# cwi-dis/cwipc_util

Hardware: NVIDIA B200
Metric: Mpoints/s for downsample+remove_outliers at 1/2/4/8 B200; % of HBM GB/s peak (higher is better)
Workload: dtype f32 keys/distances, int64 fixed-point sums, f64 statistics

## Files before the change

### cwipc_util_b200/csrc/outliers.cu

```cuda
#include <algorithm>
#include <cmath>
#include <cstdlib>
#include <cstring>
#include <mutex>

#include "device_utils.cuh"
#include "kernels.hpp"
#include "radix_sort.hpp"

namespace cwcu {

namespace {

constexpr int KG_MAX_LEVELS = 14;

struct GridParams {
    float gmin[3];
    float inv_h;
    float h;
    float rc;
    float rc_far;
    int second_min;
    int second_max;
    int gdim[3];
    int idxbits;
    int top_level;
    int bands;
    int band_bits;
    int xdim;
    uint32_t table_off[KG_MAX_LEVELS];
};
struct BandLut {
    uint8_t rank[256];
};

__host__ __device__ __forceinline__ int level_dim(int gdim, int level) { return ((gdim - 1) >> level) + 1; }

__device__ __forceinline__ uint32_t table_index(const GridParams &gp, int level, uint32_t x, uint32_t y, uint32_t z) {
    const uint32_t dx = (uint32_t)level_dim(gp.gdim[0], level), dy = (uint32_t)level_dim(gp.gdim[1], level);
    return gp.table_off[level] + (z * dy + y) * dx + x;
}

__device__ __forceinline__ uint64_t spread3(uint32_t v) {
    uint64_t x = v & 0x1fffffu;
    x = (x | x << 32) & 0x1f00000000ffffull;
    x = (x | x << 16) & 0x1f0000ff0000ffull;
    x = (x | x << 8) & 0x100f00f00f00f00full;
    x = (x | x << 4) & 0x10c30c30c30c30c3ull;
    x = (x | x << 2) & 0x1249249249249249ull;
    return x;
}
__device__ __forceinline__ uint32_t compact3(uint64_t x) {
    x &= 0x1249249249249249ull;
    x = (x | x >> 2) & 0x10c30c30c30c30c3ull;
    x = (x | x >> 4) & 0x100f00f00f00f00full;
    x = (x | x >> 8) & 0x1f0000ff0000ffull;
    x = (x | x >> 16) & 0x1f00000000ffffull;
    x = (x | x >> 32) & 0x1fffffull;
    return (uint32_t)x;
}
__device__ __forceinline__ uint64_t morton3(uint32_t x, uint32_t y, uint32_t z) { return (spread3(x) << 2) | (spread3(y) << 1) | spread3(z); }

__device__ __forceinline__ float cell_u(float x, float gmin, float inv_h) { return __fmul_rn(__fsub_rn(x, gmin), inv_h); }
__device__ __forceinline__ int cell_of(float u, int gdim) { return min(max((int)floorf(u), 0), gdim - 1); }

__device__ __forceinline__ float dist2(const Point16 &a, const Point16 &b) {
    const float dx = __fsub_rn(a.x, b.x), dy = __fsub_rn(a.y, b.y), dz = __fsub_rn(a.z, b.z);
    return __fadd_rn(__fadd_rn(__fmul_rn(dx, dx), __fmul_rn(dy, dy)), __fmul_rn(dz, dz));
}

__global__ void __launch_bounds__(256) knn_keygen_kernel(const cwipc_point *__restrict__ pts, uint32_t n, const __grid_constant__ GridParams gp, const __grid_constant__ BandLut lut,
                                                          uint64_t *__restrict__ keys, uint2 *__restrict__ table, uint32_t table_words2) {
    for (uint32_t i = blockIdx.x * blockDim.x + threadIdx.x; i < table_words2; i += gridDim.x * blockDim.x) table[i] = make_uint2(0u, 0u);
    for (uint32_t i = blockIdx.x * blockDim.x + threadIdx.x; i < n; i += gridDim.x * blockDim.x) {
        const Point16 p = ld_point_stream(pts, i);
        uint32_t cx = cell_of(cell_u(p.x, gp.gmin[0], gp.inv_h), gp.xdim);
        const uint32_t cy = cell_of(cell_u(p.y, gp.gmin[1], gp.inv_h), gp.gdim[1]);
        const uint32_t cz = cell_of(cell_u(p.z, gp.gmin[2], gp.inv_h), gp.gdim[2]);
        if (gp.bands > 1) cx += (uint32_t)lut.rank[pt_tile(p)] << gp.band_bits;
        keys[i] = (morton3(cx, cy, cz) << gp.idxbits) | i;
    }
}

__global__ void __launch_bounds__(256) knn_layout_kernel(const uint64_t *__restrict__ sorted, uint32_t n, GridParams gp, const cwipc_point *__restrict__ pts,
                                                          cwipc_point *__restrict__ spts, uint2 *__restrict__ table) {
    const uint64_t idxmask = (1ull << gp.idxbits) - 1ull;
    for (uint32_t i = blockIdx.x * blockDim.x + threadIdx.x; i < n; i += gridDim.x * blockDim.x) {
        const uint64_t word = sorted[i];
        st_point(spts, i, ld_point(pts, (size_t)(word & idxmask)));
        const uint64_t code = word >> gp.idxbits;
        int top;
        uint64_t prev = 0;
        if (i == 0) {
            top = gp.top_level;
        } else {
            prev = sorted[i - 1] >> gp.idxbits;
            const uint64_t diff = code ^ prev;
            top = diff ? min((63 - __clzll((long long)diff)) / 3, gp.top_level) : -1;
        }
        if (top >= 0) {
            const uint32_t cx = compact3(code >> 2), cy = compact3(code >> 1), cz = compact3(code);
            const uint32_t px = compact3(prev >> 2), py = compact3(prev >> 1), pz = compact3(prev);
            for (int l = 0; l <= top; l++) {
                table[table_index(gp, l, cx >> l, cy >> l, cz >> l)].x = i;
                if (i > 0) table[table_index(gp, l, px >> l, py >> l, pz >> l)].y = i;
            }
// ... 24 lines not shown
        if (!done) {
            if (t0 == 0) t0 = clock64();
            else if (clock64() - t0 > 4000000000ll) __trap();
        }
    } while (!done);
}
__device__ __forceinline__ void bulk_g2s(void *dst, const void *src, uint32_t bytes, uint64_t *bar) {
    asm volatile("cp.async.bulk.shared::cluster.global.mbarrier::complete_tx::bytes [%0], [%1], %2, [%3];" ::"r"(smem_u32(dst)), "l"(src), "r"(bytes),
                 "r"(smem_u32(bar))
                 : "memory");
}

template <int N>
__device__ __forceinline__ void bitonic_sort_asc(float (&a)[N]) {
#pragma unroll
    for (int k = 2; k <= N; k <<= 1) {
#pragma unroll
        for (int j = k >> 1; j > 0; j >>= 1) {
#pragma unroll
            for (int i = 0; i < N; i++) {
                const int l = i ^ j;
                if (l > i) {
                    const float lo = fminf(a[i], a[l]), hi = fmaxf(a[i], a[l]);
                    const bool up = (i & k) == 0;
                    a[i] = up ? lo : hi;
                    a[l] = up ? hi : lo;
                }
            }
        }
    }
}
template <int N>
__device__ __forceinline__ void bitonic_merge_asc(float (&a)[N]) {
#pragma unroll
    for (int j = N >> 1; j > 0; j >>= 1) {
#pragma unroll
        for (int i = 0; i < N; i++) {
            const int l = i ^ j;
            if (l > i) {
                const float lo = fminf(a[i], a[l]), hi = fmaxf(a[i], a[l]);
                a[i] = lo;
                a[l] = hi;
            }
        }
    }
}

struct FarEntry {
    uint32_t q;
    float bound;
};

constexpr int KT_WARPS = 2;
constexpr int KT_THREADS = KT_WARPS * 32;
constexpr int KT_CH = 128;
constexpr int KT_STAGES = 2;
constexpr int KT_GROUP_LEVEL = 2;
constexpr int KT_GROUP_SPAN = 1 << KT_GROUP_LEVEL;
constexpr int KT_MAXR = (KT_GROUP_SPAN + 2) * (KT_GROUP_SPAN + 2) * (KT_GROUP_SPAN + 2);
constexpr int KT_BUF = 16;
constexpr int KT_BLOCKS_PER_SM = 12;

struct __align__(128) KnnWarpSmem {
    Point16 cand[KT_STAGES][KT_CH];
    float buf[KT_BUF][32];
    uint2 ranges[KT_MAXR];
    uint64_t mbar[KT_STAGES];
    float pbox[7];
    uint32_t xoff;
    uint32_t cursor;
};

__device__ __forceinline__ float warp_min(float v) {
#pragma unroll
    for (int o = 16; o > 0; o >>= 1) v = fminf(v, __shfl_xor_sync(FULL_MASK, v, o));
    return v;
}
__device__ __forceinline__ float warp_max(float v) {
#pragma unroll
    for (int o = 16; o > 0; o >>= 1) v = fmaxf(v, __shfl_xor_sync(FULL_MASK, v, o));
    return v;
}

template <int KCAP>
__global__ void __launch_bounds__(KT_THREADS, KT_BLOCKS_PER_SM) knn_tile_kernel(const cwipc_point *__restrict__ spts, const uint64_t *__restrict__ sorted, uint32_t n, GridParams gp, int kk, int k,
                                                               const uint2 *__restrict__ table, float *__restrict__ dist_out, float *__restrict__ kth_out, uint32_t nquery,
                                                               FarEntry *__restrict__ far_list, uint32_t *__restrict__ far_count) {
    extern __shared__ __align__(128) unsigned char knn_smem_raw[];
    constexpr int B = KCAP < KT_BUF ? KCAP : KT_BUF;
    const unsigned lane = lane_id(), warp = threadIdx.x >> 5;
    KnnWarpSmem &ws = reinterpret_cast<KnnWarpSmem *>(knn_smem_raw)[warp];
    const unsigned lt = lanemask_lt();
    if (lane == 0) {
#pragma unroll
        for (int st = 0; st < KT_STAGES; st++) mbar_init(&ws.mbar[st], 1);
        mbar_fence_init();
    }
    __syncwarp();
    uint32_t phase_bits = 0;

    const uint32_t warps_total = (gridDim.x * blockDim.x) >> 5;
    const uint64_t idxmask = (1ull << gp.idxbits) - 1ull;
    const int extra = KCAP - kk;
    const uint32_t nitems = (n + 31u) >> 5;
    const Point16 *spts16 = reinterpret_cast<const Point16 *>(spts);
    const float rc = gp.rc;
    const float reach = (rc - 0.01f) * gp.h;
    const float reach2 = reach * reach * 0.999999f;

    for (uint32_t item = (blockIdx.x * blockDim.x + threadIdx.x) >> 5; item < nitems; item += warps_total) {
        const uint32_t qi = item * 32u + lane;
        const uint32_t qs = qi < n ? qi : n - 1u;
        const uint64_t word = sorted[qs];
        const bool active = qi < n && (uint32_t)(word & idxmask) < nquery;
        const uint64_t code = word >> gp.idxbits;
        const Point16 q = spts16[qs];
        const float ux = cell_u(q.x, gp.gmin[0], gp.inv_h), uy = cell_u(q.y, gp.gmin[1], gp.inv_h), uz = cell_u(q.z, gp.gmin[2], gp.inv_h);
        const uint32_t band = gp.bands > 1 ? (compact3(code >> 2) >> gp.band_bits) : 0u;

        const uint64_t node2 = code >> (3 * KT_GROUP_LEVEL);
        const uint64_t prev_node2 = __shfl_up_sync(FULL_MASK, node2, 1);
        const unsigned heads = __ballot_sync(FULL_MASK, (lane == 0) || (node2 != prev_node2));
        const int m = __popc(heads);
        const int ord = __popc(heads & (lt | (1u << lane))) - 1;

        for (int g = 0; g < m; g++) {
            const bool live = active && ord == g;

            const float lox = warp_min(live ? ux : INFINITY), loy = warp_min(live ? uy : INFINITY), loz = warp_min(live ? uz : INFINITY);
            const float hix = warp_max(live ? ux : -INFINITY), hiy = warp_max(live ? uy : -INFINITY), hiz = warp_max(live ? uz : -INFINITY);
            uint32_t nr = 0, total = 0;
            const uint32_t xoff = gp.bands > 1 ? (__reduce_max_sync(FULL_MASK, live ? band : 0u) << gp.band_bits) : 0u;
            if (lox <= hix) {
                const int cx0 = max((int)floorf(lox - rc), 0), cx1 = min((int)floorf(hix + rc), gp.xdim - 1);
                const int cy0 = max((int)floorf(loy - rc), 0), cy1 = min((int)floorf(hiy + rc), gp.gdim[1] - 1);
                const int cz0 = max((int)floorf(loz - rc), 0), cz1 = min((int)floorf(hiz + rc), gp.gdim[2] - 1);
                const int nbx = cx1 - cx0 + 1, nby = cy1 - cy0 + 1, nbz = cz1 - cz0 + 1;
                const int nb = nbx * nby * nbz;
                const float rc2 = rc * rc;
                for (int shell = 0; shell < 2; shell++) {
                    for (int t0 = 0; t0 < nb; t0 += 32) {
                        const int t = t0 + (int)lane;
                        uint2 r = make_uint2(0u, 0u);
                        if (t < nb) {
                            const int ix = cx0 + t % nbx, iy = cy0 + (t / nbx) % nby, iz = cz0 + t / (nbx * nby);
                            const float dx = fmaxf(fmaxf((float)ix - hix, lox - (float)(ix + 1)), 0.f);
                            const float dy = fmaxf(fmaxf((float)iy - hiy, loy - (float)(iy + 1)), 0.f);
                            const float dz = fmaxf(fmaxf((float)iz - hiz, loz - (float)(iz + 1)), 0.f);
                            const float dd = dx * dx + dy * dy + dz * dz;
                            if (shell == 0 ? dd == 0.f : (dd > 0.f && dd <= rc2)) r = table[table_index(gp, 0, (uint32_t)ix + xoff, (uint32_t)iy, (uint32_t)iz)];
                        }
                        const unsigned has = __ballot_sync(FULL_MASK, r.y > r.x);
                        if (r.y > r.x) ws.ranges[nr + __popc(has & lt)] = r;
                        nr += __popc(has);
                        total += warp_sum(r.y - r.x);
                    }
                }
            }
            __syncwarp();

            float best[KCAP];
#pragma unroll
            for (int j = 0; j < KCAP; j++) best[j] = (j < extra) ? -INFINITY : INFINITY;
            float tau = live ? INFINITY : -INFINITY;
            uint32_t bcnt = 0;

            const uint32_t nchunks = (total + KT_CH - 1) / KT_CH;
            uint32_t ri = 0, roff = 0;
            auto fill = [&](int st, uint32_t chunk) {
                const uint32_t cnt = min((uint32_t)KT_CH, total - chunk * KT_CH);
                mbar_arrive_expect_tx(&ws.mbar[st], cnt * 16u);
                uint32_t filled = 0;
                while (filled < cnt) {
                    const uint2 r = ws.ranges[ri];
                    const uint32_t len = r.y - r.x;
                    const uint32_t take = min(len - roff, cnt - filled);
                    bulk_g2s(&ws.cand[st][filled], spts16 + r.x + roff, take * 16u, &ws.mbar[st]);
                    filled += take;
                    roff += take;
                    if (roff == len) {
                        ri++;
                        roff = 0;
                    }
                }
            };
            if (lane == 0 && nchunks > 0) {
                fill(0, 0);
                if (nchunks > 1) fill(1, 1);
            }
            for (uint32_t chunk = 0; chunk < nchunks; chunk++) {
                const int st = (int)(chunk & 1u);
                mbar_wait(&ws.mbar[st], (phase_bits >> st) & 1u);
                phase_bits ^= 1u << st;
                const uint32_t cnt = min((uint32_t)KT_CH, total - chunk * KT_CH);
                const bool last_chunk = chunk + 1 == nchunks;
                for (uint32_t c = 0; c < cnt; c += 4) {
                    if (c + 4 <= cnt) {
#pragma unroll
                        for (int u = 0; u < 4; u++) {
                            const Point16 cand = ws.cand[st][c + u];
                            const float d2 = dist2(q, cand);
                            if (d2 < tau) {
                                ws.buf[bcnt][lane] = d2;
                                bcnt++;
                            }
                        }
                    } else {
                        for (uint32_t u = c; u < cnt; u++) {
                            const float d2 = dist2(q, ws.cand[st][u]);
                            if (d2 < tau) {
                                ws.buf[bcnt][lane] = d2;
                                bcnt++;
                            }
                        }
                    }
                    const bool finish = last_chunk && c + 4 >= cnt;
                    if (finish || __any_sync(FULL_MASK, bcnt > (uint32_t)(B - 4))) {
                        float s[B];
#pragma unroll
                        for (int j = 0; j < B; j++) s[j] = ((uint32_t)j < bcnt) ? ws.buf[j][lane] : INFINITY;
                        bitonic_sort_asc<B>(s);
#pragma unroll
                        for (int j = 0; j < B; j++) best[KCAP - 1 - j] = fminf(best[KCAP - 1 - j], s[j]);
                        bitonic_merge_asc<KCAP>(best);
                        bcnt = 0;
                        if (live) tau = best[KCAP - 1];
                    }
                }
                __syncwarp();
                if (lane == 0 && chunk + 2 < nchunks) fill(st, chunk + 2);
            }

            const float worst = best[KCAP - 1];
            const bool done = live && (gp.top_level == 0 || worst <= reach2);
            const unsigned fm = __ballot_sync(FULL_MASK, live && !done);
            if (fm) {
                uint32_t slot = 0;
                if (lane == (unsigned)(__ffs(fm) - 1)) slot = atomicAdd(far_count, (uint32_t)__popc(fm));
                slot = __shfl_sync(FULL_MASK, slot, __ffs(fm) - 1);
                if (live && !done) {
                    FarEntry e;
                    e.q = qi;
                    e.bound = worst;
                    far_list[slot + __popc(fm & lt)] = e;
                }
            }
            if (!done) continue;
            double sum = 0.0;
#pragma unroll
            for (int j = 0; j < KCAP; j++)
                if (j > extra) sum += sqrt((double)best[j]);
            dist_out[(size_t)(word & idxmask)] = (float)(sum / (double)k);
            if (kth_out) kth_out[(size_t)(word & idxmask)] = worst;
        }
        __syncwarp();
    }
}


template <int KCAP>
__global__ void __launch_bounds__(KT_THREADS, KT_BLOCKS_PER_SM) knn_second_kernel(const cwipc_point *__restrict__ spts, const uint64_t *__restrict__ sorted, GridParams gp, int kk, int k,
                                                                 const uint2 *__restrict__ table, float *__restrict__ dist_out, float *__restrict__ kth_out,
                                                                 const FarEntry *__restrict__ far_list, const uint32_t *__restrict__ far_count, uint32_t second_from,
                                                                 FarEntry *__restrict__ far_list2, uint32_t *__restrict__ far_count2) {
    extern __shared__ __align__(128) unsigned char knn_smem_raw[];
    constexpr int B = KCAP < KT_BUF ? KCAP : KT_BUF;
    const unsigned lane = lane_id(), warp = threadIdx.x >> 5;
    KnnWarpSmem &ws = reinterpret_cast<KnnWarpSmem *>(knn_smem_raw)[warp];
    const unsigned lt = lanemask_lt();
    if (lane == 0) {
#pragma unroll
        for (int st = 0; st < KT_STAGES; st++) mbar_init(&ws.mbar[st], 1);
        mbar_fence_init();
    }
    __syncwarp();
    uint32_t phase_bits = 0;

    const uint32_t warps_total = (gridDim.x * blockDim.x) >> 5;
    const uint64_t idxmask = (1ull << gp.idxbits) - 1ull;
    const int extra = KCAP - kk;
    const uint32_t nent = *far_count;
    if (nent < second_from) return;
    const uint32_t nitems = (nent + 31u) >> 5;
    const Point16 *spts16 = reinterpret_cast<const Point16 *>(spts);

    for (uint32_t item = (blockIdx.x * blockDim.x + threadIdx.x) >> 5; item < nitems; item += warps_total) {
        const uint32_t ei = item * 32u + lane;
        const bool valid = ei < nent;
        const FarEntry ent = far_list[valid ? ei : nent - 1u];
        const uint64_t word = sorted[ent.q];
        const uint64_t code = word >> gp.idxbits;
        const Point16 q = spts16[ent.q];
        const float need = sqrtf(ent.bound) * gp.inv_h * 1.000001f + 0.02f;
        const uint64_t node2 = code >> (3 * KT_GROUP_LEVEL);
        bool active = valid && need <= gp.rc_far;
        {
            const unsigned peers = __match_any_sync(FULL_MASK, node2) & __ballot_sync(FULL_MASK, active);
            active = active && __popc(peers) >= gp.second_min;
        }
        {
            const unsigned fm = __ballot_sync(FULL_MASK, valid && !active);
            if (fm) {
                uint32_t slot = 0;
                if (lane == (unsigned)(__ffs(fm) - 1)) slot = atomicAdd(far_count2, (uint32_t)__popc(fm));
                slot = __shfl_sync(FULL_MASK, slot, __ffs(fm) - 1);
                if (valid && !active) far_list2[slot + __popc(fm & lt)] = ent;
            }
        }
        if (!__any_sync(FULL_MASK, active)) continue;

        const uint64_t prev_node2 = __shfl_up_sync(FULL_MASK, node2, 1);
        const unsigned heads = __ballot_sync(FULL_MASK, (lane == 0) || (node2 != prev_node2));
        const int m = __popc(heads);
        const int ord = __popc(heads & (lt | (1u << lane))) - 1;

        for (int g = 0; g < m; g++) {
            const bool live = active && ord == g;
            if (!__any_sync(FULL_MASK, live)) continue;
            {
                const float ux = cell_u(q.x, gp.gmin[0], gp.inv_h), uy = cell_u(q.y, gp.gmin[1], gp.inv_h), uz = cell_u(q.z, gp.gmin[2], gp.inv_h);
                const float lx = warp_min(live ? ux : INFINITY), ly = warp_min(live ? uy : INFINITY), lz = warp_min(live ? uz : INFINITY);
                const float hx = warp_max(live ? ux : -INFINITY), hy = warp_max(live ? uy : -INFINITY), hz = warp_max(live ? uz : -INFINITY);
                const float pr = warp_max(live ? need : 0.f);
                const uint32_t band = gp.bands > 1 ? __reduce_max_sync(FULL_MASK, live ? (compact3(code >> 2) >> gp.band_bits) : 0u) : 0u;
                if (lane == 0) {
                    ws.pbox[0] = lx; ws.pbox[1] = ly; ws.pbox[2] = lz;
                    ws.pbox[3] = hx; ws.pbox[4] = hy; ws.pbox[5] = hz;
                    ws.pbox[6] = pr;
                    ws.xoff = band << gp.band_bits;
                    ws.cursor = 0u;
                }
            }
            __syncwarp();

            float best[KCAP];
#pragma unroll
            for (int j = 0; j < KCAP; j++) best[j] = (j < extra) ? -INFINITY : INFINITY;
            float tau = live ? __uint_as_float(__float_as_uint(ent.bound) + 1u) : -INFINITY;
// ... 347 lines not shown
        const int cl = node_level - 1;
        const uint32_t chx = 2u * node_x + ((lane >> 2) & 1u), chy = 2u * node_y + ((lane >> 1) & 1u), chz = 2u * node_z + (lane & 1u);
        push_nodes(expand, cl, chx, chy, chz, thr);
        __syncwarp();
    }
}

__global__ void __launch_bounds__(256) knn_queue_all_kernel(const uint64_t *__restrict__ sorted, uint32_t n, int idxbits, uint32_t nquery, FarEntry *__restrict__ far_list,
                                                             uint32_t *__restrict__ far_count) {
    const uint64_t idxmask = (1ull << idxbits) - 1ull;
    const unsigned lane = lane_id();
    const uint32_t rounds = (n + blockDim.x * gridDim.x - 1) / (blockDim.x * gridDim.x);
    for (uint32_t r = 0; r < rounds; r++) {
        const uint32_t i = (r * gridDim.x + blockIdx.x) * blockDim.x + threadIdx.x;
        const bool query = i < n && (uint32_t)(sorted[i] & idxmask) < nquery;
        const unsigned m = __ballot_sync(FULL_MASK, query);
        if (m == 0u) continue;
        uint32_t first = 0;
        if (lane == (unsigned)(__ffs(m) - 1)) first = atomicAdd(far_count, (uint32_t)__popc(m));
        first = __shfl_sync(FULL_MASK, first, __ffs(m) - 1);
        if (query) {
            FarEntry e;
            e.q = i;
            e.bound = INFINITY;
            far_list[first + __popc(m & lanemask_lt())] = e;
        }
    }
}

__device__ __forceinline__ FarStart far_start(const Point16 q, uint64_t code, const GridParams &gp, int kk, const uint2 *__restrict__ table, uint32_t band, float &limit) {
    const unsigned lane = lane_id();
    const uint32_t cx = compact3(code >> 2), cy = compact3(code >> 1), cz = compact3(code);
    const int root_level = gp.bands > 1 ? gp.band_bits : gp.top_level;
    const float slack = 0.01f * gp.h;
    const float qq[3] = {q.x, q.y, q.z};
    bool enough = false;
    float far2 = INFINITY;
    if ((int)lane <= root_level) {
        const int l = (int)lane;
        const uint32_t ax = cx >> l, ay = cy >> l, az = cz >> l;
        const uint2 r = table[table_index(gp, l, ax, ay, az)];
        if (r.y - r.x >= (uint32_t)kk) {
            enough = true;
            const float pitch = ldexpf(gp.h, l);
            const uint32_t lx = ax - (band << (gp.band_bits - l));
            const float lo[3] = {gp.gmin[0] + (float)lx * pitch, gp.gmin[1] + (float)ay * pitch, gp.gmin[2] + (float)az * pitch};
            far2 = 0.f;
#pragma unroll
            for (int a = 0; a < 3; a++) {
                const float d = fmaxf(qq[a] - lo[a], (lo[a] + pitch) - qq[a]) + slack;
                far2 += d * d;
            }
        }
    }
    FarStart st;
    st.level = -1;
    st.x = st.y = st.z = 0u;
    const unsigned m = __ballot_sync(FULL_MASK, enough);
    if (m != 0u) limit = fminf(limit, __shfl_sync(FULL_MASK, far2, __ffs(m) - 1) * 1.0001f);
    if (!(limit < INFINITY)) return st;
    const float rcells = sqrtf(limit) * gp.inv_h * 1.000001f + 0.02f;
    const float u[3] = {cell_u(q.x, gp.gmin[0], gp.inv_h), cell_u(q.y, gp.gmin[1], gp.inv_h), cell_u(q.z, gp.gmin[2], gp.inv_h)};
    const int dim[3] = {gp.xdim, gp.gdim[1], gp.gdim[2]};
    uint32_t lo[3], hi[3];
#pragma unroll
    for (int a = 0; a < 3; a++) {
        lo[a] = (uint32_t)min(max((int)floorf(u[a] - rcells), 0), dim[a] - 1);
        hi[a] = (uint32_t)min(max((int)floorf(u[a] + rcells), 0), dim[a] - 1);
    }
    lo[0] += band << gp.band_bits;
    hi[0] += band << gp.band_bits;
    for (int l = 0; l < root_level; l++) {
        if ((hi[0] >> l) - (lo[0] >> l) <= 1u && (hi[1] >> l) - (lo[1] >> l) <= 1u && (hi[2] >> l) - (lo[2] >> l) <= 1u) {
            st.level = l;
            st.x = lo[0] >> l;
            st.y = lo[1] >> l;
            st.z = lo[2] >> l;
            break;
        }
    }
    return st;
}

template <int KPL>
__global__ void __launch_bounds__(KF_THREADS) knn_far_kernel(const cwipc_point *__restrict__ spts, const uint64_t *__restrict__ sorted, uint32_t n, const __grid_constant__ GridParams gp, int kk, int k,
                                                              const uint2 *__restrict__ table, float *__restrict__ dist_out, float *__restrict__ kth_out,
                                                              const FarEntry *__restrict__ far_list, const uint32_t *__restrict__ far_count, uint32_t second_from,
                                                              uint32_t leaf_points, bool far_start_enabled) {
    __shared__ __align__(16) FarNode s_stack[KF_WARPS][KF_STACK];
    const unsigned lane = lane_id(), warp = threadIdx.x >> 5;
    if (far_count[0] >= second_from) {
        far_list += (size_t)n + 64;
        far_count += 1;
    }
    const uint32_t nentries = *far_count;
    const uint32_t warps_total = (gridDim.x * blockDim.x) >> 5;
    const uint64_t idxmask = (1ull << gp.idxbits) - 1ull;
    const Point16 *spts16 = reinterpret_cast<const Point16 *>(spts);
    for (uint32_t ei = (blockIdx.x * blockDim.x + threadIdx.x) >> 5; ei < nentries; ei += warps_total) {
        const FarEntry ent = far_list[ei];
        float v[KPL];
        const uint64_t code = sorted[ent.q] >> gp.idxbits;
        const uint32_t band = gp.bands > 1 ? (compact3(code >> 2) >> gp.band_bits) : 0u;
        const Point16 q = spts16[ent.q];
        float limit = ent.bound;
        FarStart start;
        start.level = -1;
        start.x = start.y = start.z = 0u;
        if (far_start_enabled) start = far_start(q, code, gp, kk, table, band, limit);
        dfs_knn<KPL>(q, limit, spts16, n, gp, kk, table, leaf_points, s_stack[warp], v, band, start);
        double sq[KPL];
#pragma unroll
        for (int j = 0; j < KPL; j++) sq[j] = sqrt((double)v[j]);
        double *s_sq = reinterpret_cast<double *>(s_stack[warp]);
        __syncwarp();
#pragma unroll
        for (int j = 0; j < KPL; j++) s_sq[j * 32 + (int)lane] = sq[j];
        __syncwarp();
        double sum = 0.0;
        for (int e = 1; e <= k; e++) sum += s_sq[e];
        const float kth = list_element<KPL>(v, kk - 1);
        __syncwarp();
        if (lane == 0) {
            const size_t orig = (size_t)(sorted[ent.q] & idxmask);
            dist_out[orig] = (float)(sum / (double)k);
            if (kth_out) kth_out[orig] = kth;
        }
    }
}

template <int KPL>
__global__ void __launch_bounds__(KF_THREADS) knn_list_kernel(const cwipc_point *__restrict__ spts, uint32_t n, GridParams gp, int kk, const uint2 *__restrict__ table,
                                                               const cwipc_point *__restrict__ queries, const float *__restrict__ limits, uint32_t nq, float *__restrict__ lists,
                                                               uint32_t leaf_points) {
    __shared__ __align__(16) FarNode s_stack[KF_WARPS][KF_STACK];
    const unsigned lane = lane_id(), warp = threadIdx.x >> 5;
    const uint32_t warps_total = (gridDim.x * blockDim.x) >> 5;
    const Point16 *spts16 = reinterpret_cast<const Point16 *>(spts);
    for (uint32_t qi = (blockIdx.x * blockDim.x + threadIdx.x) >> 5; qi < nq; qi += warps_total) {
        float v[KPL];
        dfs_knn<KPL>(ld_point(queries, qi), limits ? limits[qi] : INFINITY, spts16, n, gp, kk, table, leaf_points, s_stack[warp], v);
#pragma unroll
        for (int j = 0; j < KPL; j++) {
            const int e = j * 32 + (int)lane;
            if (e < kk) lists[(size_t)qi * kk + e] = v[j];
        }
    }
}

__global__ void __launch_bounds__(128) knn_merge_lists_kernel(const float *__restrict__ lists, uint32_t nlists, uint32_t nq, int kk, int k, float *__restrict__ mean,
                                                               float *__restrict__ kth_out) {
    const uint32_t q = blockIdx.x * blockDim.x + threadIdx.x;
    if (q >= nq) return;
    uint32_t head[16];
    for (uint32_t l = 0; l < nlists; l++) head[l] = 0;
    double sum = 0.0;
    float last = 0.f;
    for (int e = 0; e < kk; e++) {
        float best = INFINITY;
        uint32_t arg = 0;
        for (uint32_t l = 0; l < nlists; l++) {
            if (head[l] < (uint32_t)kk) {
                const float x = lists[((size_t)l * nq + q) * kk + head[l]];
                if (x < best) {
                    best = x;
                    arg = l;
                }
            }
        }
        head[arg]++;
        if (e > 0) sum += sqrt((double)best);
        last = best;
    }
    mean[q] = (float)(sum / (double)k);
    if (kth_out) kth_out[q] = last;
}

constexpr int ST_BLOCKS = 256;
constexpr int ST_THREADS = 256;

__global__ void __launch_bounds__(ST_THREADS) stats_kernel(const float *__restrict__ dist, uint32_t n, double *__restrict__ partial) {
    __shared__ double s_sum[ST_THREADS], s_sq[ST_THREADS];
    double sum = 0.0, sq = 0.0;
    for (uint32_t i = blockIdx.x * ST_THREADS + threadIdx.x; i < n; i += ST_BLOCKS * ST_THREADS) {
        const float d = dist[i];
        sum += (double)d;
        sq += (double)__fmul_rn(d, d);
    }
    s_sum[threadIdx.x] = sum;
    s_sq[threadIdx.x] = sq;
    __syncthreads();
    for (int o = ST_THREADS / 2; o > 0; o >>= 1) {
        if ((int)threadIdx.x < o) {
// ... 123 lines not shown
    }
    return b;
}

unsigned stream_grid(size_t n, int dev) {
    return (unsigned)std::max<size_t>(1, std::min(div_up(n, 256), (size_t)sm_count(dev) * 8));
}

float env_float(const char *name, float dflt, float lo, float hi) {
    const char *e = getenv(name);
    if (!e || !*e) return dflt;
    const float v = (float)atof(e);
    return (v >= lo && v <= hi) ? v : dflt;
}

struct GridPlan {
    GridParams gp;
    size_t table_entries = 0;
};

GridPlan choose_grid(const float gmin[3], const float gmax[3], size_t n, int k, float hint_spacing, int bands = 1) {
    static const float pitch_factor = env_float("CWIPC_CUDA_KNN_PITCH", 1.0f, 0.05f, 20.f);
    static const float rc = env_float("CWIPC_CUDA_KNN_RC", 1.0f, 0.25f, 1.0f);
    static const float rc_far = env_float("CWIPC_CUDA_KNN_RC_FAR", 2.0f, 0.f, 8.f);
    GridPlan plan;
    GridParams &gp = plan.gp;
    memset(&gp, 0, sizeof(gp));
    const double ext[3] = {(double)gmax[0] - gmin[0], (double)gmax[1] - gmin[1], (double)gmax[2] - gmin[2]};
    double spacing = hint_spacing > 0.f ? (double)hint_spacing : 0.0;
    const double longest = std::max(ext[0], std::max(ext[1], ext[2]));
    if (!(spacing > 0.0)) {
        const double area = 2.0 * (ext[0] * ext[1] + ext[1] * ext[2] + ext[2] * ext[0]);
        const double per_band = std::max(1.0, (double)n / (double)bands);
        if (area > 0.0) spacing = std::sqrt(area / per_band);
        else if (longest > 0.0) spacing = longest / per_band;
        else spacing = 1.0;
    }
    double h = spacing * std::sqrt((double)(k + 1) / 3.14159265358979) * (double)pitch_factor;
    gp.idxbits = std::max(1, bit_length((uint64_t)n - 1));
    const int rank_bits = bands > 1 ? bit_length((uint64_t)bands - 1) : 0;
    const int max_axis_bits = std::min(13, (64 - gp.idxbits) / 3) - rank_bits;
    if (max_axis_bits < 2) throw CudaError{cudaErrorInvalidValue, "remove_outliers: too many points and tiles for one search index"};
    if (!(h > 0.0) || !std::isfinite(h)) h = 1.0;
    static const float cells_per_point = env_float("CWIPC_CUDA_KNN_CELLS_PER_POINT", 16.f, 0.25f, 1024.f);
    static const float max_cells_log2 = env_float("CWIPC_CUDA_KNN_MAX_CELLS_LOG2", 27.f, 16.f, 30.f);
    const double cell_cap = std::min(std::max((double)cells_per_point * (double)n, 65536.0), std::ldexp(1.0, (int)max_cells_log2)) / (bands > 1 ? 2.0 * (double)bands : 1.0);
    while (true) {
        const double cells = (std::floor(ext[0] / h) + 2) * (std::floor(ext[1] / h) + 2) * (std::floor(ext[2] / h) + 2);
        if (longest / h < (double)((1 << max_axis_bits) - 1) && cells <= cell_cap) break;
        h *= 1.25;
    }
    gp.h = (float)h;
    gp.inv_h = 1.0f / gp.h;
    gp.rc = rc;
    gp.rc_far = rc_far;
    gp.second_min = (int)env_float("CWIPC_CUDA_KNN_SECOND_MIN", 2.f, 1.f, 32.f);
    gp.second_max = (int)env_float("CWIPC_CUDA_KNN_SECOND_MAX", 150.f, 1.f, 1.0e6f);
    int maxdim = 1;
    for (int a = 0; a < 3; a++) {
        gp.gmin[a] = gmin[a];
        gp.gdim[a] = std::max(1, std::min((int)std::floor(ext[a] / (double)gp.h) + 2, 1 << max_axis_bits));
        maxdim = std::max(maxdim, gp.gdim[a]);
    }
    gp.top_level = bit_length((uint64_t)maxdim - 1);
    gp.bands = std::max(1, bands);
    gp.xdim = gp.gdim[0];
    gp.band_bits = gp.top_level;
    if (gp.bands > 1) {
        gp.band_bits = std::max(gp.top_level, KT_GROUP_LEVEL);
        gp.gdim[0] = ((gp.bands - 1) << gp.band_bits) + gp.xdim;
        gp.top_level = gp.band_bits + rank_bits;
    }
    size_t off = 0;
    for (int l = 0; l <= gp.top_level; l++) {
        gp.table_off[l] = (uint32_t)off;
        off += (size_t)level_dim(gp.gdim[0], l) * level_dim(gp.gdim[1], l) * level_dim(gp.gdim[2], l);
    }
    plan.table_entries = off;
    return plan;
}

uint32_t far_leaf_points() {
    static const uint32_t v = (uint32_t)env_float("CWIPC_CUDA_KNN_LEAF", 128.f, 1.f, 65536.f);
    return v;
}

template <int KCAP>
void run_knn(const cwipc_point *spts, const uint64_t *sorted, size_t n, const GridParams &gp, int k, const uint2 *table, float *d_dist, float *d_kth, size_t nquery,
             FarEntry *far_list, uint32_t *far_count, int dev, cudaStream_t s) {
    const int kk = k + 1;
    const size_t smem = sizeof(KnnWarpSmem) * KT_WARPS;
    static std::once_flag once[64];
    std::call_once(once[dev & 63], [&] {
        CWCU_CHECK(cudaFuncSetAttribute(knn_tile_kernel<KCAP>, cudaFuncAttributeMaxDynamicSharedMemorySize, (int)smem));
        CWCU_CHECK(cudaFuncSetAttribute(knn_second_kernel<KCAP>, cudaFuncAttributeMaxDynamicSharedMemorySize, (int)smem));
    });
    const size_t nitems = div_up(n, (size_t)32);
    const unsigned grid = (unsigned)std::max<size_t>(1, std::min(div_up(nitems, (size_t)KT_WARPS), (size_t)sm_count(dev) * KT_BLOCKS_PER_SM));
    tune_kernel(knn_tile_kernel<KCAP>, CHAIN_CARVEOUT);
    launch("knn_tile_kernel", s, 28 * (size_t)n, [&] {
        knn_tile_kernel<KCAP><<<grid, KT_THREADS, smem, s>>>(spts, sorted, (uint32_t)n, gp, kk, k, table, d_dist, d_kth, (uint32_t)nquery, far_list, far_count);
    });
    if (gp.top_level == 0) return;
    uint32_t second_from = 0xffffffffu;
    static const float second_from_n = env_float("CWIPC_CUDA_KNN_SECOND_FROM_N", 262144.f, 0.f, 4.0e9f);
    if (gp.rc_far > gp.rc && (double)std::min(nquery, n) >= (double)second_from_n) {
        static const float share = env_float("CWIPC_CUDA_KNN_SECOND_SHARE", 0.f, 0.f, 1.f);
        second_from = (uint32_t)std::max(1.0, std::ceil((double)share * (double)std::min(nquery, n)));
        tune_kernel(knn_second_kernel<KCAP>, CHAIN_CARVEOUT);
        launch("knn_second_kernel", s, (size_t)0, [&] {
            knn_second_kernel<KCAP><<<(unsigned)sm_count(dev) * KT_BLOCKS_PER_SM, KT_THREADS, smem, s>>>(spts, sorted, gp, kk, k, table, d_dist, d_kth, far_list, far_count, second_from,
                                                                                                         far_list + (n + 64), far_count + 1);
        });
    }
    constexpr int KPL = KCAP > 32 ? 2 : 1;
    tune_kernel(knn_far_kernel<KPL>, CHAIN_CARVEOUT);
    launch("knn_far_kernel", s, (size_t)0, [&] {
        static const bool far_start_on = env_float("CWIPC_CUDA_KNN_FAR_START", 1.f, 0.f, 1.f) != 0.f;
        knn_far_kernel<KPL><<<(unsigned)sm_count(dev) * 8, KF_THREADS, 0, s>>>(spts, sorted, (uint32_t)n, gp, kk, k, table, d_dist, d_kth, far_list, far_count, second_from, far_leaf_points(),
                                                                               far_start_on);
    });
}

template <int KPL>
void run_knn_wide(const cwipc_point *spts, const uint64_t *sorted, size_t n, const GridParams &gp, int k, const uint2 *table, float *d_dist, float *d_kth, size_t nquery,
                  FarEntry *far_list, uint32_t *far_count, int dev, cudaStream_t s) {
    launch("knn_queue_all_kernel", s, 8 * n, [&] {
        knn_queue_all_kernel<<<stream_grid(n, dev), 256, 0, s>>>(sorted, (uint32_t)n, gp.idxbits, (uint32_t)nquery, far_list, far_count);
    });
    launch("knn_far_kernel", s, (size_t)0, [&] {
        static const bool far_start_on = env_float("CWIPC_CUDA_KNN_FAR_START", 1.f, 0.f, 1.f) != 0.f;
        knn_far_kernel<KPL><<<(unsigned)sm_count(dev) * 8, KF_THREADS, 0, s>>>(spts, sorted, (uint32_t)n, gp, k + 1, k, table, d_dist, d_kth, far_list, far_count, 0xffffffffu, far_leaf_points(),
                                                                               far_start_on);
    });
}

struct KnnIndex {
    GridParams gp;
    Scratch keys_a, keys_b, spts, table;
    const uint64_t *sorted = nullptr;
    uint32_t *far_count = nullptr;
};

void build_index(KnnIndex &ix, const cwipc_point *in, size_t n, int k, float hint_spacing, const float *bounds, int dev, cudaStream_t s, const BandLut *lut = nullptr, int bands = 1) {
    float gmin[3], gmax[3];
    if (bounds) {
        for (int a = 0; a < 3; a++) {
            gmin[a] = bounds[a];
            gmax[a] = bounds[3 + a];
        }
    } else {
        global_bbox(in, n, gmin, gmax, dev, s);
    }
    for (int a = 0; a < 3; a++)
        if (!std::isfinite(gmin[a]) || !std::isfinite(gmax[a])) throw CudaError{cudaErrorInvalidValue, "remove_outliers: pointcloud contains non-finite coordinates"};
    const GridPlan plan = choose_grid(gmin, gmax, n, k, hint_spacing, lut ? bands : 1);
    BandLut band_lut;
    if (lut) band_lut = *lut;
    else memset(&band_lut, 0, sizeof(band_lut));
    ix.gp = plan.gp;
    const GridParams &gp = ix.gp;
    int axis_bits = 1;
    for (int a = 0; a < 3; a++) axis_bits = std::max(axis_bits, bit_length((uint64_t)gp.gdim[a] - 1));
    const int keybits = 3 * axis_bits;

    ix.keys_a = Scratch(n * sizeof(uint64_t), s);
    ix.keys_b = Scratch(n * sizeof(uint64_t), s);
    ix.spts = Scratch(n * sizeof(cwipc_point), s);
    ix.table = Scratch((plan.table_entries + 2) * sizeof(uint2), s);
    ix.far_count = reinterpret_cast<uint32_t *>(ix.table.as<uint2>() + plan.table_entries);
    tune_kernel(knn_keygen_kernel, CHAIN_CARVEOUT);
    tune_kernel(knn_layout_kernel, CHAIN_CARVEOUT);
    launch("knn_keygen_kernel", s, 24 * (size_t)n, [&] {
        knn_keygen_kernel<<<stream_grid(std::max(n, plan.table_entries / 4), dev), 256, 0, s>>>(in, (uint32_t)n, gp, band_lut, ix.keys_a.as<uint64_t>(), ix.table.as<uint2>(),
                                                                                                 (uint32_t)(plan.table_entries + 2));
    });
    ix.sorted = radix_sort_u64(ix.keys_a.as<uint64_t>(), ix.keys_b.as<uint64_t>(), n, gp.idxbits, gp.idxbits + keybits, dev, s);

    launch("knn_layout_kernel", s, 48 * (size_t)n, [&] {
        knn_layout_kernel<<<stream_grid(n, dev), 256, 0, s>>>(ix.sorted, (uint32_t)n, gp, in, ix.spts.as<cwipc_point>(), ix.table.as<uint2>());
    });
}

void check_k(int k, size_t n) {
    if (k < 1) throw CudaError{cudaErrorInvalidValue, "remove_outliers: kNeighbors must be >= 1"};
    if (k > KNN_MAX_K) throw CudaError{cudaErrorInvalidValue, "remove_outliers: kNeighbors > " + std::to_string(KNN_MAX_K) + " is not supported by libcwipc_util_cuda"};
    (void)n;
}

}

namespace {
void knn_mean_distances_banded(const cwipc_point *in, size_t n, int k, float hint_spacing, const float *bounds, float *d_dist, int dev, cudaStream_t s, float *d_kth, size_t nquery,
                               const BandLut *lut, int bands) {
    if (n == 0) return;
    check_k(k, n);
    if ((size_t)k >= n) throw CudaError{cudaErrorInvalidValue, "remove_outliers: needs more than kNeighbors points"};
    KnnIndex ix;
    build_index(ix, in, n, k, hint_spacing, bounds, dev, s, lut, bands);
    Scratch far_list(2 * (n + 64) * sizeof(FarEntry), s);
    const int kk = k + 1;
    auto go = [&](auto kcap) {
        run_knn<decltype(kcap)::value>(ix.spts.as<cwipc_point>(), ix.sorted, n, ix.gp, k, ix.table.as<uint2>(), d_dist, d_kth, std::min(nquery, n), far_list.as<FarEntry>(),
                                       ix.far_count, dev, s);
    };
    auto go_wide = [&](auto kpl) {
        run_knn_wide<decltype(kpl)::value>(ix.spts.as<cwipc_point>(), ix.sorted, n, ix.gp, k, ix.table.as<uint2>(), d_dist, d_kth, std::min(nquery, n), far_list.as<FarEntry>(), ix.far_count,
                                           dev, s);
    };
    if (kk <= 8) go(std::integral_constant<int, 8>{});
    else if (kk <= 16) go(std::integral_constant<int, 16>{});
    else if (kk <= 32) go(std::integral_constant<int, 32>{});
    else if (kk <= 64) go(std::integral_constant<int, 64>{});
    else if (kk <= 128) go_wide(std::integral_constant<int, 4>{});
    else if (kk <= 256) go_wide(std::integral_constant<int, 8>{});
    else go_wide(std::integral_constant<int, 16>{});
// ... 193 lines not shown
```

Measured before the change: 8644.

## Seed kNN pruning threshold, merge contiguous cell ranges, add debug counters

Seeds the per-query pruning threshold tau with a finite radius bound instead of infinity, so candidates beyond the reach of the later far or second pass are rejected early and fewer buffer flushes happen. Cell enumeration now walks z-fastest in a single shell pass and coalesces adjacent table ranges into one, which cuts the number of bulk copies. A templated counting variant gated by an env var reports per-warp statistics. The risks are changed candidate ordering and possible correctness issues if the seed bound is wrong for some queries.

```diff
diff --git a/cwipc_util_b200/csrc/outliers.cu b/cwipc_util_b200/csrc/outliers.cu
--- a/cwipc_util_b200/csrc/outliers.cu
+++ b/cwipc_util_b200/csrc/outliers.cu
@@ -1,5 +1,6 @@
 #include <algorithm>
 #include <cmath>
+#include <cstdio>
 #include <cstdlib>
 #include <cstring>
 #include <mutex>
@@ -22,6 +23,7 @@
     float rc_far;
     int second_min;
     int second_max;
+    float seed2;
     int gdim[3];
     int idxbits;
     int top_level;
@@ -212,10 +214,10 @@
     return v;
 }
 
-template <int KCAP>
+template <int KCAP, bool COUNT = false>
 __global__ void __launch_bounds__(KT_THREADS, KT_BLOCKS_PER_SM) knn_tile_kernel(const cwipc_point *__restrict__ spts, const uint64_t *__restrict__ sorted, uint32_t n, GridParams gp, int kk, int k,
                                                                const uint2 *__restrict__ table, float *__restrict__ dist_out, float *__restrict__ kth_out, uint32_t nquery,
-                                                               FarEntry *__restrict__ far_list, uint32_t *__restrict__ far_count) {
+                                                               FarEntry *__restrict__ far_list, uint32_t *__restrict__ far_count, unsigned long long *__restrict__ counters) {
     extern __shared__ __align__(128) unsigned char knn_smem_raw[];
     constexpr int B = KCAP < KT_BUF ? KCAP : KT_BUF;
     const unsigned lane = lane_id(), warp = threadIdx.x >> 5;
@@ -237,6 +239,8 @@
     const float rc = gp.rc;
     const float reach = (rc - 0.01f) * gp.h;
     const float reach2 = reach * reach * 0.999999f;
+    const float seed = fmaxf(gp.seed2, __uint_as_float(__float_as_uint(reach2) + 1u));
+    unsigned long long n_items = 0, n_groups = 0, n_ranges = 0, n_parks = 0, n_flushes = 0;
 
     for (uint32_t item = (blockIdx.x * blockDim.x + threadIdx.x) >> 5; item < nitems; item += warps_total) {
         const uint32_t qi = item * 32u + lane;
@@ -268,31 +272,44 @@
                 const int nbx = cx1 - cx0 + 1, nby = cy1 - cy0 + 1, nbz = cz1 - cz0 + 1;
                 const int nb = nbx * nby * nbz;
                 const float rc2 = rc * rc;
-                for (int shell = 0; shell < 2; shell++) {
-                    for (int t0 = 0; t0 < nb; t0 += 32) {
-                        const int t = t0 + (int)lane;
-                        uint2 r = make_uint2(0u, 0u);
-                        if (t < nb) {
-                            const int ix = cx0 + t % nbx, iy = cy0 + (t / nbx) % nby, iz = cz0 + t / (nbx * nby);
-                            const float dx = fmaxf(fmaxf((float)ix - hix, lox - (float)(ix + 1)), 0.f);
-                            const float dy = fmaxf(fmaxf((float)iy - hiy, loy - (float)(iy + 1)), 0.f);
-                            const float dz = fmaxf(fmaxf((float)iz - hiz, loz - (float)(iz + 1)), 0.f);
-                            const float dd = dx * dx + dy * dy + dz * dz;
-                            if (shell == 0 ? dd == 0.f : (dd > 0.f && dd <= rc2)) r = table[table_index(gp, 0, (uint32_t)ix + xoff, (uint32_t)iy, (uint32_t)iz)];
-                        }
-                        const unsigned has = __ballot_sync(FULL_MASK, r.y > r.x);
-                        if (r.y > r.x) ws.ranges[nr + __popc(has & lt)] = r;
-                        nr += __popc(has);
-                        total += warp_sum(r.y - r.x);
+                uint32_t last_end = 0xffffffffu;
+                for (int t0 = 0; t0 < nb; t0 += 32) {
+                    const int t = t0 + (int)lane;
+                    uint2 r = make_uint2(0u, 0u);
+                    if (t < nb) {
+                        const int iz = cz0 + t % nbz, iy = cy0 + (t / nbz) % nby, ix = cx0 + t / (nbz * nby);
+                        const float dx = fmaxf(fmaxf((float)ix - hix, lox - (float)(ix + 1)), 0.f);
+                        const float dy = fmaxf(fmaxf((float)iy - hiy, loy - (float)(iy + 1)), 0.f);
+                        const float dz = fmaxf(fmaxf((float)iz - hiz, loz - (float)(iz + 1)), 0.f);
+                        if (dx * dx + dy * dy + dz * dz <= rc2) r = table[table_index(gp, 0, (uint32_t)ix + xoff, (uint32_t)iy, (uint32_t)iz)];
                     }
+                    const bool has_r = r.y > r.x;
+                    const unsigned has = __ballot_sync(FULL_MASK, has_r);
+                    if (has == 0u) continue;
+                    const unsigned before = has & lt;
+                    const uint32_t prev_y = __shfl_sync(FULL_MASK, r.y, before ? 31 - __clz(before) : 0);
+                    const bool joins = has_r && r.x == (before ? prev_y : last_end);
+                    const unsigned joinm = __ballot_sync(FULL_MASK, joins);
+                    const unsigned heads = has & ~joinm;
+                    const unsigned after = has & ~lt & ~(1u << lane);
+                    const int slot = (int)nr + __popc(heads & (lt | (1u << lane))) - 1;
+                    if (has_r && !joins) ws.ranges[slot].x = r.x;
+                    if (has_r && (after == 0u || !((joinm >> (__ffs(after) - 1)) & 1u))) ws.ranges[slot].y = r.y;
+                    nr += __popc(heads);
+                    last_end = __shfl_sync(FULL_MASK, r.y, 31 - __clz(has));
+                    total += warp_sum(r.y - r.x);
                 }
             }
             __syncwarp();
+            if (COUNT) {
+                n_groups++;
+                n_ranges += nr;
+            }
 
             float best[KCAP];
 #pragma unroll
             for (int j = 0; j < KCAP; j++) best[j] = (j < extra) ? -INFINITY : INFINITY;
-            float tau = live ? INFINITY : -INFINITY;
+            float tau = live ? seed : -INFINITY;
             uint32_t bcnt = 0;
 
             const uint32_t nchunks = (total + KT_CH - 1) / KT_CH;
@@ -353,8 +370,12 @@
 #pragma unroll
                         for (int j = 0; j < B; j++) best[KCAP - 1 - j] = fminf(best[KCAP - 1 - j], s[j]);
                         bitonic_merge_asc<KCAP>(best);
+                        if (COUNT) {
+                            n_parks += bcnt;
+                            n_flushes++;
+                        }
                         bcnt = 0;
-                        if (live) tau = best[KCAP - 1];
+                        tau = fminf(tau, best[KCAP - 1]);
                     }
                 }
                 __syncwarp();
@@ -384,6 +405,16 @@
             if (kth_out) kth_out[(size_t)(word & idxmask)] = worst;
         }
         __syncwarp();
+        if (COUNT) n_items++;
+    }
+    if (COUNT) {
+        if (lane == 0) {
+            atomicAdd(&counters[0], n_items);
+            atomicAdd(&counters[1], n_groups);
+            atomicAdd(&counters[2], n_ranges);
+            atomicAdd(&counters[4], n_flushes);
+        }
+        atomicAdd(&counters[3], n_parks);
     }
 }
 
@@ -1228,14 +1259,45 @@
     });
     const size_t nitems = div_up(n, (size_t)32);
     const unsigned grid = (unsigned)std::max<size_t>(1, std::min(div_up(nitems, (size_t)KT_WARPS), (size_t)sm_count(dev) * KT_BLOCKS_PER_SM));
-    tune_kernel(knn_tile_kernel<KCAP>, CHAIN_CARVEOUT);
-    launch("knn_tile_kernel", s, 28 * (size_t)n, [&] {
-        knn_tile_kernel<KCAP><<<grid, KT_THREADS, smem, s>>>(spts, sorted, (uint32_t)n, gp, kk, k, table, d_dist, d_kth, (uint32_t)nquery, far_list, far_count);
-    });
+    static const float second_from_n = env_float("CWIPC_CUDA_KNN_SECOND_FROM_N", 262144.f, 0.f, 4.0e9f);
+    const bool second_scan = gp.top_level > 0 && gp.rc_far > gp.rc && (double)std::min(nquery, n) >= (double)second_from_n;
+    static const float seed_factor = env_float("CWIPC_CUDA_KNN_SEED", 1.0f, 0.f, 100.f);
+    GridParams gpm = gp;
+    gpm.seed2 = INFINITY;
+    if (seed_factor > 0.f && gp.top_level > 0) {
+        double seed = (double)seed_factor * ((double)gp.rc - 0.01) * (double)gp.h;
+        if (second_scan) seed = std::max(seed, (double)gp.rc_far * (double)gp.h);
+        gpm.seed2 = (float)(seed * seed * (1.0 + 1e-5));
+    }
+    static const bool debug_knn = getenv("CWIPC_CUDA_DEBUG_KNN") != nullptr;
+    if (debug_knn) {
+        static std::once_flag once_dbg[64];
+        std::call_once(once_dbg[dev & 63], [&] { CWCU_CHECK(cudaFuncSetAttribute(knn_tile_kernel<KCAP, true>, cudaFuncAttributeMaxDynamicSharedMemorySize, (int)smem)); });
+        Scratch counters(8 * sizeof(unsigned long long), s);
+        CWCU_CHECK(cudaMemsetAsync(counters.p, 0, 8 * sizeof(unsigned long long), s));
+        tune_kernel(knn_tile_kernel<KCAP, true>, CHAIN_CARVEOUT);
+        launch("knn_tile_kernel", s, 28 * (size_t)n, [&] {
+            knn_tile_kernel<KCAP, true><<<grid, KT_THREADS, smem, s>>>(spts, sorted, (uint32_t)n, gpm, kk, k, table, d_dist, d_kth, (uint32_t)nquery, far_list, far_count,
+                                                                     counters.as<unsigned long long>());
+        });
+        unsigned long long h[8];
+        uint32_t nfar = 0;
+        CWCU_CHECK(cudaMemcpyAsync(h, counters.p, sizeof(h), cudaMemcpyDeviceToHost, s));
+        CWCU_CHECK(cudaMemcpyAsync(&nfar, far_count, sizeof(nfar), cudaMemcpyDeviceToHost, s));
+        stream_sync(s);
+        const double items = (double)std::max(1ull, h[0]);
+        fprintf(stderr, "knn_tile_kernel n=%zu k=%d seed=%g reach2=%g: %llu warp items, %llu groups, per warp item: %.2f ranges, %.1f parked per lane, %.2f flushes; %u queued\n", n, k,
+                (double)gpm.seed2, (double)(((gp.rc - 0.01f) * gp.h) * ((gp.rc - 0.01f) * gp.h) * 0.999999f), h[0], h[1], (double)h[2] / items, (double)h[3] / items / 32.0,
+                (double)h[4] / items, nfar);
+    } else {
+        tune_kernel(knn_tile_kernel<KCAP>, CHAIN_CARVEOUT);
+        launch("knn_tile_kernel", s, 28 * (size_t)n, [&] {
+            knn_tile_kernel<KCAP><<<grid, KT_THREADS, smem, s>>>(spts, sorted, (uint32_t)n, gpm, kk, k, table, d_dist, d_kth, (uint32_t)nquery, far_list, far_count, nullptr);
+        });
+    }
     if (gp.top_level == 0) return;
     uint32_t second_from = 0xffffffffu;
-    static const float second_from_n = env_float("CWIPC_CUDA_KNN_SECOND_FROM_N", 262144.f, 0.f, 4.0e9f);
-    if (gp.rc_far > gp.rc && (double)std::min(nquery, n) >= (double)second_from_n) {
+    if (second_scan) {
         static const float share = env_float("CWIPC_CUDA_KNN_SECOND_SHARE", 0.f, 0.f, 1.f);
         second_from = (uint32_t)std::max(1.0, std::ceil((double)share * (double)std::min(nquery, n)));
         tune_kernel(knn_second_kernel<KCAP>, CHAIN_CARVEOUT);
```

Result: faster. 8762 (median of 6 runs) (+1.4%).

## Add expanding-ring grid search before DFS fallback in far kNN kernel

Applied to the files above, without the earlier changes.

For far-list queries, the kernel now first searches level-0 grid cells in concentric shells around the query cell, up to a default of 6 rings. It gathers non-empty cell ranges warp-cooperatively, flattens them with a prefix scan, and absorbs candidate distances into the k-list. If the next shell's minimum distance exceeds the current k-th bound, the result is final and the hierarchical DFS is skipped; otherwise the bound is tightened and DFS runs as before. The goal is to avoid stack-based tree traversal for most far queries, at the risk of wasted ring work when queries still fall back to DFS.

```diff
diff --git a/cwipc_util_b200/csrc/outliers.cu b/cwipc_util_b200/csrc/outliers.cu
--- a/cwipc_util_b200/csrc/outliers.cu
+++ b/cwipc_util_b200/csrc/outliers.cu
@@ -897,11 +897,114 @@
     return st;
 }
 
+constexpr int RING_CELLS = 4;
+static_assert(KF_STACK * sizeof(FarNode) >= 32 * RING_CELLS * sizeof(uint2), "the range list of ring_knn lives in the stack memory");
+
+template <int KPL>
+__device__ __forceinline__ bool ring_knn(const Point16 q, uint64_t code, float &limit, const Point16 *__restrict__ spts16, const GridParams &gp, int kk,
+                                         const uint2 *__restrict__ table, float (&v)[KPL], uint32_t band, int ring_max, uint2 *list) {
+    const unsigned lane = lane_id();
+    const float slack = 0.01f * gp.h;
+    const uint32_t xoff = band << gp.band_bits;
+    const int c[3] = {(int)(compact3(code >> 2) - xoff), (int)compact3(code >> 1), (int)compact3(code)};
+    const int dim[3] = {gp.xdim, gp.gdim[1], gp.gdim[2]};
+    const float qq[3] = {q.x, q.y, q.z};
+    auto axis_gap = [&](int a, int i) {
+        const float lo = gp.gmin[a] + (float)i * gp.h;
+        return fmaxf(fmaxf(lo - qq[a], qq[a] - (lo + gp.h)) - slack, 0.f);
+    };
+#pragma unroll
+    for (int j = 0; j < KPL; j++) v[j] = INFINITY;
+    float tau = INFINITY;
+    for (int r = 1; r <= ring_max; r++) {
+        const int side = 2 * r + 1, face = side * side, belt = 8 * r;
+        const int nring = 24 * r * r + 2, ncells = nring + (r == 1 ? 1 : 0);
+        const float inv_side = 1.f / (float)side, inv_belt = 1.f / (float)belt, inv_run = 1.f / (float)(2 * r);
+        for (int t0 = 0; t0 < ncells; t0 += 32 * RING_CELLS) {
+            const float thr = fminf(tau, limit);
+            uint2 rg[RING_CELLS];
+#pragma unroll
+            for (int u = 0; u < RING_CELLS; u++) {
+                const int t = t0 + 32 * u + (int)lane;
+                int o[3] = {0, 0, 0};
+                if (t < 2 * face) {
+                    const int zf = t >= face ? 1 : 0, w = t - zf * face;
+                    const int row = (int)(((float)w + 0.5f) * inv_side);
+                    o[0] = w - row * side - r;
+                    o[1] = row - r;
+                    o[2] = zf ? r : -r;
+                } else if (t < nring) {
+                    const int w = t - 2 * face;
+                    const int layer = (int)(((float)w + 0.5f) * inv_belt), p = w - layer * belt;
+                    const int run = (int)(((float)p + 0.5f) * inv_run), e = p - run * 2 * r;
+                    o[0] = run == 0 ? e - r : run == 1 ? r : run == 2 ? r - e : -r;
+                    o[1] = run == 0 ? -r : run == 1 ? e - r : run == 2 ? r : r - e;
+                    o[2] = layer - (r - 1);
+                }
+                rg[u] = make_uint2(0u, 0u);
+                if (t < ncells && (unsigned)(c[0] + o[0]) < (unsigned)dim[0] && (unsigned)(c[1] + o[1]) < (unsigned)dim[1] && (unsigned)(c[2] + o[2]) < (unsigned)dim[2]) {
+                    float mind2 = 0.f;
+#pragma unroll
+                    for (int a = 0; a < 3; a++) {
+                        const float d = axis_gap(a, c[a] + o[a]);
+                        mind2 += d * d;
+                    }
+                    if (mind2 * 0.9999f <= thr) rg[u] = table[table_index(gp, 0, (uint32_t)(c[0] + o[0]) + xoff, (uint32_t)(c[1] + o[1]), (uint32_t)(c[2] + o[2]))];
+                }
+            }
+            uint32_t nr = 0;
+#pragma unroll
+            for (int u = 0; u < RING_CELLS; u++) {
+                const bool has = rg[u].y > rg[u].x;
+                const unsigned hm = __ballot_sync(FULL_MASK, has);
+                if (has) list[nr + __popc(hm & lanemask_lt())] = rg[u];
+                nr += (uint32_t)__popc(hm);
+            }
+            __syncwarp();
+            for (uint32_t r0 = 0; r0 < nr; r0 += 32) {
+                const uint2 cell = r0 + lane < nr ? list[r0 + lane] : make_uint2(0u, 0u);
+                const uint32_t len = cell.y - cell.x;
+                uint32_t incl = len;
+#pragma unroll
+                for (int s = 1; s < 32; s <<= 1) {
+                    const uint32_t y = __shfl_up_sync(FULL_MASK, incl, s);
+                    if ((int)lane >= s) incl += y;
+                }
+                const uint32_t total = __shfl_sync(FULL_MASK, incl, 31);
+                const uint32_t shift = cell.x - (incl - len);
+                for (uint32_t base = 0; base < total; base += 32) {
+                    const uint32_t i = base + lane;
+                    int j = 0;
+#pragma unroll
+                    for (int s = 16; s > 0; s >>= 1)
+                        if (__shfl_sync(FULL_MASK, incl, j + s - 1) <= i) j += s;
+                    const uint32_t sh = __shfl_sync(FULL_MASK, shift, j);
+                    float d2 = INFINITY;
+                    if (i < total) d2 = dist2(q, spts16[sh + i]);
+                    const bool pass = d2 < tau && d2 <= limit;
+                    const unsigned pm = __ballot_sync(FULL_MASK, pass);
+                    if (pm) tau = list_absorb<KPL>(v, d2, pass, pm, kk, lane);
+                }
+            }
+            __syncwarp();
+        }
+        float dmin = INFINITY;
+#pragma unroll
+        for (int a = 0; a < 3; a++) {
+            if (c[a] - r > 0) dmin = fminf(dmin, axis_gap(a, c[a] - r - 1));
+            if (c[a] + r < dim[a] - 1) dmin = fminf(dmin, axis_gap(a, c[a] + r + 1));
+        }
+        if (dmin == INFINITY || dmin * dmin * 0.9999f > fminf(tau, limit)) return true;
+    }
+    limit = fminf(limit, tau);
+    return false;
+}
+
 template <int KPL>
 __global__ void __launch_bounds__(KF_THREADS) knn_far_kernel(const cwipc_point *__restrict__ spts, const uint64_t *__restrict__ sorted, uint32_t n, const __grid_constant__ GridParams gp, int kk, int k,
                                                               const uint2 *__restrict__ table, float *__restrict__ dist_out, float *__restrict__ kth_out,
                                                               const FarEntry *__restrict__ far_list, const uint32_t *__restrict__ far_count, uint32_t second_from,
-                                                              uint32_t leaf_points, bool far_start_enabled) {
+                                                              uint32_t leaf_points, bool far_start_enabled, int ring_max) {
     __shared__ __align__(16) FarNode s_stack[KF_WARPS][KF_STACK];
     const unsigned lane = lane_id(), warp = threadIdx.x >> 5;
     if (far_count[0] >= second_from) {
@@ -923,7 +1026,11 @@
         start.level = -1;
         start.x = start.y = start.z = 0u;
         if (far_start_enabled) start = far_start(q, code, gp, kk, table, band, limit);
-        dfs_knn<KPL>(q, limit, spts16, n, gp, kk, table, leaf_points, s_stack[warp], v, band, start);
+        bool found = false;
+        if constexpr (KPL <= 2) {
+            if (ring_max > 0) found = ring_knn<KPL>(q, code, limit, spts16, gp, kk, table, v, band, ring_max, reinterpret_cast<uint2 *>(s_stack[warp]));
+        }
+        if (!found) dfs_knn<KPL>(q, limit, spts16, n, gp, kk, table, leaf_points, s_stack[warp], v, band, start);
         double sq[KPL];
 #pragma unroll
         for (int j = 0; j < KPL; j++) sq[j] = sqrt((double)v[j]);
@@ -1213,6 +1320,11 @@
 
 uint32_t far_leaf_points() {
     static const uint32_t v = (uint32_t)env_float("CWIPC_CUDA_KNN_LEAF", 128.f, 1.f, 65536.f);
+    return v;
+}
+
+int far_ring_max() {
+    static const int v = env_float("CWIPC_CUDA_KNN_FAR_RING", 1.f, 0.f, 1.f) != 0.f ? (int)env_float("CWIPC_CUDA_KNN_RING_MAX", 6.f, 1.f, 64.f) : 0;
     return v;
 }
 
@@ -1249,7 +1361,7 @@
     launch("knn_far_kernel", s, (size_t)0, [&] {
         static const bool far_start_on = env_float("CWIPC_CUDA_KNN_FAR_START", 1.f, 0.f, 1.f) != 0.f;
         knn_far_kernel<KPL><<<(unsigned)sm_count(dev) * 8, KF_THREADS, 0, s>>>(spts, sorted, (uint32_t)n, gp, kk, k, table, d_dist, d_kth, far_list, far_count, second_from, far_leaf_points(),
-                                                                               far_start_on);
+                                                                               far_start_on, far_ring_max());
     });
 }
 
@@ -1262,7 +1374,7 @@
     launch("knn_far_kernel", s, (size_t)0, [&] {
         static const bool far_start_on = env_float("CWIPC_CUDA_KNN_FAR_START", 1.f, 0.f, 1.f) != 0.f;
         knn_far_kernel<KPL><<<(unsigned)sm_count(dev) * 8, KF_THREADS, 0, s>>>(spts, sorted, (uint32_t)n, gp, k + 1, k, table, d_dist, d_kth, far_list, far_count, 0xffffffffu, far_leaf_points(),
-                                                                               far_start_on);
+                                                                               far_start_on, 0);
     });
 }
 
```

Measured after the change: 8706 before, 8566 after (median of 6 runs). 0.984x the previous value.
